# scitix/arks

Hardware: AMD Instinct MI355X
Metric: output_tok_s (higher is better)
Workload: dtype bf16; 1 GPU; model=qwen2.5-7b, global_batch=64, seq_len=1024, parallelism=dp1

## Files before the change

### arks_amd/ops/__init__.py

```python

from __future__ import annotations

import os
from typing import Callable, NamedTuple

import torch

from . import ref

_C = None
_C_ERR: str | None = None


def _load_extension():
    global _C, _C_ERR
    if _C is not None or _C_ERR is not None:
        return _C
    try:
        from . import _load

        _C = _load.C
    except Exception as e:
        _C_ERR = f"{type(e).__name__}: {e}"
    return _C
# ... 237 lines not shown
    return nparts


def attention_decode_paged(
    q, k_cache, v_cache, block_tables, seq_lens, scale: float,
    num_partitions: int | None = None, part_out=None, window: int = 0,
):
    if q.is_cuda:
        out = torch.empty(
            (q.shape[0], q.shape[1], q.shape[2]), dtype=q.dtype, device=q.device
        )
        num_kv_heads = k_cache.shape[1]
        if num_partitions is None:
            num_partitions = decode_num_partitions(
                q.shape[0], num_kv_heads, block_tables.shape[1]
            )
        if num_partitions > 1 and part_out is None:
            gq = q.shape[1] // num_kv_heads
            part_out = torch.empty(
                q.shape[0] * num_kv_heads * num_partitions * gq * (q.shape[2] + 2),
                dtype=torch.float32, device=q.device,
            )
        elif part_out is None:
            part_out = q.new_empty(0, dtype=torch.float32)
        _native().attention_decode_paged(
            out, q, k_cache, v_cache, block_tables, seq_lens, scale,
            part_out, num_partitions, window,
        )
        return out
    return ref.attention_decode_paged(
        q, k_cache, v_cache, block_tables, seq_lens, scale, window
    )


_EXTEND_WS: dict = {}


def _extend_ws(need: int, device):
    key = (device.index,)
    ws = _EXTEND_WS.get(key)
    if ws is None or ws.numel() < need:
        ws = torch.empty(need, dtype=torch.float32, device=device)
        _EXTEND_WS[key] = ws
    return ws


_SKINNY_WS: dict = {}
_SKINNY_WS_GEN: dict = {}


class SplitKPending:

    __slots__ = ("ws", "nsplits", "mrows", "shape", "bias", "_key", "_gen")

    def __init__(self, ws, nsplits, mrows, M, N, bias, key):
        self.ws = ws
        self.nsplits = nsplits
        self.mrows = mrows
        self.shape = (M, N)
        self.bias = bias
        self._key = key
        self._gen = _SKINNY_WS_GEN[key]

    def check_live(self) -> None:
        if _SKINNY_WS_GEN.get(self._key) != self._gen:
            raise RuntimeError(
                "stale split-K handle: another skinny GEMM has overwritten "
                "the shared workspace since this result was produced"
            )

    def materialize(self) -> torch.Tensor:
        self.check_live()
        out = torch.empty(self.shape, dtype=torch.bfloat16,
                          device=self.ws.device)
        _native().skinny_combine(out, self.ws, self.bias, self.nsplits,
                                 self.mrows)
        return out


def skinny_gemm(x, weight, bias=None, defer: bool = False):
    M, K = x.shape
    N = weight.shape[0]
    config, nsplits, k_per_split, mrows = _skinny_plan(M, N, K)
    part = (_skinny_ws(nsplits, N, mrows, x.device) if nsplits > 1
            else x.new_empty(0, dtype=torch.float32))
    if defer and nsplits > 1:
        _native().skinny_gemm_partials(part, x, weight, k_per_split, nsplits,
                                       config)
        return SplitKPending(part, nsplits, mrows, M, N, bias,
                             (x.device.index,))
    out = torch.empty((M, N), dtype=x.dtype, device=x.device)
    _native().skinny_gemm(out, part, x, weight, bias, k_per_split, nsplits,
                          config)
    return out


def _skinny_plan(M: int, N: int, K: int):
    ntiles = N // 64
    if K > N and ntiles < 128 and M > 48:
        config, mt = _SKINNY_TALLK_CONFIG, 4
        nsplits = min(-(-448 // ntiles), -(-K // 256))
    else:
        config, mt = 0, min(-(-M // 16), 4)
        nsplits = 1 if ntiles >= 384 else min(-(-512 // ntiles), -(-K // 256))
    k_per_split = -(-(-(-K // nsplits)) // 32) * 32
    nsplits = -(-K // k_per_split)
    return config, nsplits, k_per_split, 16 * mt


def _skinny_ws(nsplits: int, N: int, mrows: int, device):
    key = (device.index,)
    need = nsplits * N * mrows
    ws = _SKINNY_WS.get(key)
    if ws is None or ws.numel() < need:
        ws = torch.empty(need, dtype=torch.float32, device=device)
        _SKINNY_WS[key] = ws
    _SKINNY_WS_GEN[key] = _SKINNY_WS_GEN.get(key, 0) + 1
    return ws


_USE_SKINNY = os.environ.get("ARKS_SKINNY_GEMM", "1") == "1"
_SPLITK_FUSE = os.environ.get("ARKS_SPLITK_FUSE", "1") == "1"
_SKINNY_MAX_ELEMS = 34_000_000
_SKINNY_TALLK_MAX_ELEMS = 80_000_000
_TALLK_V = os.environ.get("ARKS_SKINNY_TALLK_V", "7").strip()
if _TALLK_V not in ("7", "8"):
    raise ValueError(
        f"ARKS_SKINNY_TALLK_V={_TALLK_V!r}: accepted values are 7 (tall-K "
        "kernel) and 8 (tall-K kernel with non-temporal W loads)"
    )
_SKINNY_TALLK_CONFIG = {"7": 1, "8": 2}[_TALLK_V]


def linear_bf16(x, weight, bias=None, defer: bool = False):
    if (
        _USE_SKINNY
        and x.is_cuda
        and x.dim() == 2
        and 1 <= x.shape[0] <= 64
        and x.dtype == torch.bfloat16
        and weight.shape[0] % 64 == 0
        and weight.shape[1] % 32 == 0
        and (weight.numel() <= _SKINNY_MAX_ELEMS
             or (weight.shape[1] > weight.shape[0]
                 and x.shape[0] > 48
                 and weight.numel() <= _SKINNY_TALLK_MAX_ELEMS))
        and weight.is_contiguous()
        and native_available()
    ):
        return skinny_gemm(x, weight, bias, defer=defer and _SPLITK_FUSE)
    import torch.nn.functional as F

    return F.linear(x, weight, bias)


W4_SKINNY_MAX_M = W8_SKINNY_MAX_M = _WQ_SKINNY_MAX_M = 64
W4_SLAB_MAX_M = 128
W8_SLAB_MAX_M = 128
_DEQUANT_WS: dict = {}


def reserve_dequant_workspace(numel: int, device) -> None:
    device = torch.device(device)
    if device.type != "cuda":
        return
    key = (device.index if device.index is not None
           else torch.cuda.current_device(),)
    ws = _DEQUANT_WS.get(key)
    if ws is None or ws.numel() < numel:
        _DEQUANT_WS[key] = torch.empty(numel, dtype=torch.bfloat16,
                                       device=device)


class _WqFormat(NamedTuple):
    name: str
    shape: Callable
    ref_linear: Callable
    ref_dequant: Callable
    slab_max_m: int


_W4 = _WqFormat(
    "w4", lambda w: (w[0].shape[0], w[0].shape[1] * 8), ref.w4_linear,
    lambda w: ref.w4_dequant(*ref.w4_unpack(w)), W4_SLAB_MAX_M)
_W8 = _WqFormat(
    "w8", lambda w: tuple(w[0].shape),
    lambda x, w, bias: ref.w8_linear(x, *w, bias),
    lambda w: ref.w8_dequant(*w), W8_SLAB_MAX_M)


# ... 388 lines not shown
```

### arks_amd/ops/csrc/bindings.cpp

```cpp
#include <torch/extension.h>

#include <c10/hip/HIPStream.h>
#include <hip/hip_runtime.h>

#include <cstring>
#include <string>
#include <vector>

namespace py = pybind11;

extern "C" {
void arks_rmsnorm(void* out, const void* input, const void* weight, float eps,
                  int rows, int hidden, hipStream_t stream);
void arks_fused_add_rmsnorm(void* out, const void* input, void* residual,
                            const void* weight, float eps, int rows, int hidden,
                            hipStream_t stream);
void arks_silu_mul(void* out, const void* gate_up, int64_t rows, int d,
                   hipStream_t stream);
int arks_pool_max_hidden();
void arks_pool_embed(void* out, void* carry, void* part, const void* x,
                     const void* residual, const void* weight,
                     const void* segs, const void* slabs, int nsegs,
                     int nslabs, float eps, int hidden, int dims,
                     int normalize, hipStream_t stream);
void arks_rope_inplace(const void* positions, void* q, void* k,
                       const void* cos_sin, int num_tokens, int head_dim,
                       int num_q_heads, int num_kv_heads, int64_t q_stride,
                       int64_t k_stride, hipStream_t stream);
void arks_reshape_and_cache(const void* k, const void* v, void* k_cache,
                            void* v_cache, const void* slot_mapping,
                            int num_tokens, int num_kv_heads, int head_dim,
                            int block_size, int64_t kv_stride, int kv_fp8,
                            hipStream_t stream);
void arks_rope_and_cache(const void* positions, void* q, void* k,
                         const void* v, void* k_cache, void* v_cache,
                         const void* slot_mapping, const void* cos_sin,
                         int num_tokens, int head_dim, int num_q_heads,
                         int num_kv_heads, int block_size, int64_t q_stride,
                         int64_t k_stride, int kv_fp8, hipStream_t stream);
void arks_attn_decode_paged(void* out, void* part_out, const void* q,
                            const void* k_cache, const void* v_cache,
                            const void* block_tables, const void* seq_lens,
                            float scale, int num_seqs, int num_q_heads,
                            int num_kv_heads, int head_dim, int max_blocks,
                            int nparts, int64_t q_stride, int kv_fp8,
                            int window, hipStream_t stream);
void arks_attn_prefill_varlen(void* out, const void* q, const void* k,
                              const void* v, const void* cu_seqlens,
                              const void* tile_info, int ntiles, float scale,
                              int num_q_heads, int num_kv_heads, int head_dim,
                              int64_t q_stride, int64_t kv_stride, int window,
                              hipStream_t stream);
void arks_attn_extend_paged(void* out, const void* q, const void* k_cache,
                            const void* v_cache, const void* block_tables,
                            const void* kv_lens, const void* cu_seqlens_q,
                            const void* tile_info, int ntiles, float scale,
                            int num_q_heads, int num_kv_heads, int head_dim,
                            int max_blocks, int64_t q_stride, int kv_fp8,
                            int window, hipStream_t stream);
void arks_attn_extend_paged2(void* out, const void* q, const void* k_cache,
                             const void* v_cache, const void* block_tables,
                             const void* kv_lens, const void* cu_seqlens_q,
                             const void* tile_info, void* part_ws, int ntiles,
                             float scale, int num_q_heads, int num_kv_heads,
                             int head_dim, int max_blocks, int64_t q_stride,
                             int window, hipStream_t stream);
void arks_attn_extend2_combine(void* out, const void* part_ws,
                               const void* combine_table,
                               const void* cu_seqlens_q, int n_split,
                               float scale, int num_q_heads, int head_dim,
                               hipStream_t stream);
void arks_quant_fp8_rows(void* out, void* inv_scale, const void* x, int rows,
                         int cols, hipStream_t stream);
void arks_rmsnorm_fp8(void* out, void* inv_scale, const void* input,
                      void* residual, const void* weight, float eps, int rows,
                      int hidden, int fused_add, hipStream_t stream);
void arks_silu_mul_fp8(void* out, void* inv_scale, const void* gate_up,
                       int rows, int d, hipStream_t stream);
void arks_skinny_gemm(void* part, void* out, const void* a, const void* w,
                      const void* bias, int m_rows, int n_total, int k_total,
                      int k_per_split, int nsplits, int64_t a_stride,
                      int config, bool combine, hipStream_t stream);
int arks_skinny_slab_rows(int m_rows, int config);
void arks_skinny_combine(void* out, const void* part, const void* bias,
                         int m_rows, int n_total, int nsplits, int mrows_pad,
                         hipStream_t stream);
void arks_splitk_add_rmsnorm(void* out, const void* part, const void* bias,
                             void* residual, const void* weight, float eps,
                             int rows, int hidden, int nsplits, int mrows_pad,
                             hipStream_t stream);
void arks_splitk_rope_and_cache(const void* positions, const void* part,
                                const void* bias, void* q_out, void* k_cache,
                                void* v_cache, const void* slot_mapping,
                                const void* cos_sin, int num_tokens,
                                int head_dim, int num_q_heads,
                                int num_kv_heads, int block_size, int nsplits,
                                int mrows_pad, int kv_fp8, hipStream_t stream);
void arks_greedy_sample(void* out, const void* logits, int rows, int vocab,
                        hipStream_t stream);
void arks_gumbel_sample(void* out, const void* logits, const void* temperatures,
                        const void* uniform, int rows, int vocab,
                        hipStream_t stream);
void arks_greedy_sample_masked(void* out, const void* logits,
                               const void* masks, const void* mask_row,
                               int rows, int vocab, int slots,
                               hipStream_t stream);
void arks_gumbel_sample_masked(void* out, const void* logits,
                               const void* temperatures, const void* uniform,
                               const void* masks, const void* mask_row,
                               int rows, int vocab, int slots,
                               hipStream_t stream);
void arks_apply_token_bitmask(void* logits, int is_fp32, const void* masks,
                              const void* mask_row, int rows, int vocab,
                              int slots, hipStream_t stream);
void arks_ar_seq_inc(void* seq, hipStream_t stream);
void arks_one_shot_allreduce(void* out, const void* src, void* mail_ptrs[8],
                             void* flag_ptrs[8], void* seq, int rank,
                             int world, int64_t n, hipStream_t stream);
void arks_moe_topk(void* weights, void* ids, const void* logits, int T,
                   int E, int k, int renorm, hipStream_t stream);
void arks_moe_mix(void* out, const void* y, const void* weights,
                  const void* ids, int T, int H, int k, int expert_base,
                  int n_local, hipStream_t stream);
void arks_moe_mix_rows(void* out, const void* y, const void* weights,
                       const void* rows, int T, int H, int k,
                       hipStream_t stream);
void arks_lora_shrink(void* h, const void* x, const void* a, const void* tiles,
                      int ntiles, int T, int K, int SR, int max_loras,
                      hipStream_t stream);
void arks_lora_expand(void* y, const void* h, const void* b, const void* tiles,
                      int ntiles, int T, int N, int R, int S, int off1,
                      int off2, int max_loras, hipStream_t stream);
void arks_w4_skinny_gemm(void* part, void* out, const void* a, const void* qw,
                         const void* scales, const void* zeros,
                         const void* bias, int m_rows, int n_total,
                         int k_total, int k_per_split, int nsplits,
                         int64_t a_stride, int nw, bool combine,
                         hipStream_t stream);
int arks_wq_slab_rows(int m_rows);
void arks_w4_dequant(void* out, const void* qw, const void* scales,
                     const void* zeros, int n_total, int k_total,
                     hipStream_t stream);
void arks_w4_moe_gemm(void* out, const void* a, const void* qw,
                      const void* scales, const void* zeros,
                      const void* counts, const void* pairs, int n_experts,
                      int t_cols, int n_pairs, int src_div, int slabs,
                      int n_total, int k_total, int nw, hipStream_t stream);
void arks_w8_skinny_gemm(void* part, void* out, const void* a, const void* w8,
                         const void* scales, const void* bias, int m_rows,
                         int n_total, int k_total, int k_per_split,
                         int nsplits, int64_t a_stride, int nw, bool combine,
                         hipStream_t stream);
void arks_w8_dequant(void* out, const void* w8, const void* scales,
                     int n_total, int k_total, hipStream_t stream);
void arks_moe_route(void* counts, void* pairs, const void* ids, int n_pairs,
                    int T, int expert_base, int n_local, hipStream_t stream);
void arks_mfma_probe(void* d, const void* a, const void* b, hipStream_t stream);
void arks_mfma_probe32(void* d, const void* a, const void* b, hipStream_t stream);
void arks_tr16_probe(void* out, int stride_bytes, hipStream_t stream);
}

namespace {

hipStream_t current_stream() {
  return c10::hip::getCurrentHIPStream().stream();
}
// ... 214 lines not shown
                             torch::Tensor cu_seqlens_q,
                             torch::Tensor tile_info, torch::Tensor part_ws,
                             double scale, int64_t window) {
  check_bf16_contig(out, "out");
  check_bf16_rowstrided(q, "q");
  check_bf16_contig(k_cache, "k_cache");
  check_bf16_contig(v_cache, "v_cache");
  TORCH_CHECK(block_tables.scalar_type() == torch::kInt32);
  TORCH_CHECK(kv_lens.scalar_type() == torch::kInt32);
  TORCH_CHECK(cu_seqlens_q.scalar_type() == torch::kInt32);
  TORCH_CHECK(tile_info.scalar_type() == torch::kInt32);
  TORCH_CHECK(tile_info.dim() == 2 && tile_info.size(1) == 4,
              "tile_info rows are (seq, q0, part, nparts)");
  const int num_q_heads = q.size(1);
  const int head_dim = q.size(2);
  const int num_kv_heads = k_cache.size(1);
  TORCH_CHECK(k_cache.size(2) == 16, "KV block size must be 16");
  TORCH_CHECK(head_dim == 64 || head_dim == 128, "head_dim must be 64 or 128");
  const int ntiles = tile_info.size(0);
  const int max_blocks = block_tables.size(1);
  void* ws = nullptr;
  if (part_ws.numel() > 0) {
    TORCH_CHECK(part_ws.scalar_type() == torch::kFloat32);
    ws = part_ws.data_ptr();
  }
  arks_attn_extend_paged2(out.data_ptr(), q.data_ptr(), k_cache.data_ptr(),
                          v_cache.data_ptr(), block_tables.data_ptr(),
                          kv_lens.data_ptr(), cu_seqlens_q.data_ptr(),
                          tile_info.data_ptr(), ws, ntiles, (float)scale,
                          num_q_heads, num_kv_heads, head_dim, max_blocks,
                          q.stride(0), (int)window, current_stream());
}

void attention_extend2_combine(torch::Tensor out, torch::Tensor part_ws,
                               torch::Tensor combine_table,
                               torch::Tensor cu_seqlens_q, double scale) {
  check_bf16_rowstrided(out, "out");
  TORCH_CHECK(part_ws.scalar_type() == torch::kFloat32);
  TORCH_CHECK(combine_table.scalar_type() == torch::kInt32 &&
              combine_table.dim() == 2 && combine_table.size(1) == 4);
  const int num_q_heads = out.size(1);
  const int head_dim = out.size(2);
  arks_attn_extend2_combine(out.data_ptr(), part_ws.data_ptr(),
                            combine_table.data_ptr(), cu_seqlens_q.data_ptr(),
                            combine_table.size(0), (float)scale, num_q_heads,
                            head_dim, current_stream());
}

const void* check_skinny_args(const torch::Tensor& out,
                              const torch::Tensor& part,
                              const torch::Tensor& a, const torch::Tensor& w,
                              const c10::optional<torch::Tensor>& bias,
                              int64_t k, int64_t nsplits, int64_t mrows,
                              bool partials_only, const char* what) {
  check_bf16_rowstrided(a, "a");
  check_bf16_contig(w, "w");
  const int64_t m = a.size(0), n = w.size(0);
  TORCH_CHECK(m >= 1 && m <= 64, what, " needs 1 <= M <= 64");
  TORCH_CHECK(n % 64 == 0 && k % 32 == 0, "N%64==0 and K%32==0 required");
  if (partials_only) {
    TORCH_CHECK(nsplits > 1, what, ": partials-only needs nsplits > 1");
  } else {
    check_bf16_contig(out, "out");
    TORCH_CHECK(out.size(0) == m && out.size(1) == n);
  }
  const void* bias_ptr = nullptr;
  if (bias.has_value()) {
    check_bf16_contig(*bias, "bias");
    TORCH_CHECK(bias->numel() == n);
    bias_ptr = bias->data_ptr();
  }
  if (nsplits > 1) {
    TORCH_CHECK(part.is_cuda() && part.scalar_type() == torch::kFloat32 &&
                part.is_contiguous() &&
                part.numel() >= (int64_t)nsplits * n * mrows,
                what, " workspace too small");
  }
  return bias_ptr;
}

void skinny_gemm_impl(torch::Tensor out, torch::Tensor part, torch::Tensor a,
                      torch::Tensor w, c10::optional<torch::Tensor> bias,
                      int64_t k_per_split, int64_t nsplits, int64_t config,
                      bool combine) {
  const int m = a.size(0), k = a.size(1), n = w.size(0);
  TORCH_CHECK(w.size(1) == k);
  TORCH_CHECK(0 <= config && config <= 2, "config in 0..2");
  TORCH_CHECK(k_per_split >= 32 && k_per_split % 32 == 0 &&
              nsplits * k_per_split >= k, "splits must cover K");
  const int mrows = arks_skinny_slab_rows(m, (int)config);
  const void* bias_ptr = check_skinny_args(out, part, a, w, bias, k, nsplits,
                                           mrows, !combine, "skinny_gemm");
  arks_skinny_gemm(nsplits > 1 ? part.data_ptr() : nullptr,
                   combine ? out.data_ptr() : nullptr, a.data_ptr(),
                   w.data_ptr(), bias_ptr, m, n, k, (int)k_per_split,
                   (int)nsplits, a.stride(0), (int)config, combine,
                   current_stream());
}

void skinny_gemm(torch::Tensor out, torch::Tensor part, torch::Tensor a,
                 torch::Tensor w, c10::optional<torch::Tensor> bias,
                 int64_t k_per_split, int64_t nsplits, int64_t config) {
  skinny_gemm_impl(out, part, a, w, bias, k_per_split, nsplits, config, true);
}

void skinny_gemm_partials(torch::Tensor part, torch::Tensor a, torch::Tensor w,
                          int64_t k_per_split, int64_t nsplits,
                          int64_t config) {
  skinny_gemm_impl(torch::Tensor(), part, a, w, c10::nullopt, k_per_split,
                   nsplits, config, false);
}

std::pair<int64_t, int64_t> check_w4_packed(const torch::Tensor& qw,
                                            const torch::Tensor& scales,
                                            const torch::Tensor& zeros) {
  TORCH_CHECK(qw.is_cuda() && qw.scalar_type() == torch::kInt32 &&
              qw.dim() == 2 && qw.is_contiguous(),
              "qweight must be contiguous int32 [N, K/8] on GPU");
  const int64_t n = qw.size(0), k = qw.size(1) * 8;
  TORCH_CHECK(k >= 128 && k % 128 == 0, "W4 needs K % 128 == 0, got K=", k);
  TORCH_CHECK(n % 64 == 0, "W4 needs N % 64 == 0, got N=", n);
  TORCH_CHECK(scales.is_cuda() && scales.scalar_type() == torch::kFloat16 &&
              scales.is_contiguous() && scales.dim() == 2 &&
              scales.size(0) == k / 128 && scales.size(1) == n,
              "scales must be contiguous f16 [K/128, N] on GPU");
  TORCH_CHECK(zeros.is_cuda() && zeros.scalar_type() == torch::kUInt8 &&
              zeros.is_contiguous() && zeros.dim() == 2 &&
              zeros.size(0) == k / 128 && zeros.size(1) == n,
              "zeros must be contiguous uint8 [K/128, N] on GPU");
  TORCH_CHECK(scales.device() == qw.device() && zeros.device() == qw.device());
  return {n, k};
}

struct WqSkinnyArgs {
  void* part;
  void* out;
  const void* bias;
};
WqSkinnyArgs check_wq_skinny(const torch::Tensor& out,
                             const torch::Tensor& part,
                             const torch::Tensor& a,
                             const c10::optional<torch::Tensor>& bias,
                             int64_t n, int64_t k, c10::Device dev,
                             int64_t k_per_split, int64_t nsplits, int64_t nw,
                             bool combine) {
  check_bf16_rowstrided(a, "a");
  TORCH_CHECK(a.dim() == 2 && a.size(1) == k, "a must be [M, K]");
  TORCH_CHECK(a.device() == dev);
  const int64_t m = a.size(0);
  TORCH_CHECK(m >= 1 && m <= 64, "wq_skinny_gemm needs 1 <= M <= 64");
  TORCH_CHECK(a.stride(0) % 8 == 0 &&
              reinterpret_cast<uintptr_t>(a.data_ptr()) % 16 == 0,
              "a rows must be 16-byte aligned");
  TORCH_CHECK((nw == 1 || nw == 2) && n % (64 * nw) == 0,
              "nw in {1, 2} with N % (64 * nw) == 0");
  TORCH_CHECK(nsplits >= 1 && k_per_split >= 128 && k_per_split % 128 == 0 &&
              nsplits * k_per_split >= k && (nsplits - 1) * k_per_split < k,
              "splits of a multiple of 128 must cover K exactly");
  WqSkinnyArgs r{nullptr, nullptr, nullptr};
  if (combine) {
    check_bf16_contig(out, "out");
    TORCH_CHECK(out.dim() == 2 && out.size(0) == m && out.size(1) == n);
    r.out = out.data_ptr();
    if (bias.has_value()) {
      check_bf16_contig(*bias, "bias");
      TORCH_CHECK(bias->numel() == n);
      r.bias = bias->data_ptr();
    }
  } else {
    TORCH_CHECK(nsplits > 1, "partials-only needs nsplits > 1");
  }
  if (nsplits > 1) {
    TORCH_CHECK(part.is_cuda() && part.scalar_type() == torch::kFloat32 &&
                part.is_contiguous() &&
                part.numel() >= nsplits * n * arks_wq_slab_rows((int)m) &&
                reinterpret_cast<uintptr_t>(part.data_ptr()) % 16 == 0,
                "wq_skinny_gemm workspace too small");
    r.part = part.data_ptr();
  }
  return r;
}

void w4_skinny_gemm_impl(torch::Tensor out, torch::Tensor part,
                         torch::Tensor a, torch::Tensor qw,
                         torch::Tensor scales, torch::Tensor zeros,
                         c10::optional<torch::Tensor> bias,
                         int64_t k_per_split, int64_t nsplits, int64_t nw,
                         bool combine) {
  const auto [n, k] = check_w4_packed(qw, scales, zeros);
  const auto p = check_wq_skinny(out, part, a, bias, n, k, qw.device(),
                                 k_per_split, nsplits, nw, combine);
  arks_w4_skinny_gemm(p.part, p.out, a.data_ptr(), qw.data_ptr(),
                      scales.data_ptr(), zeros.data_ptr(), p.bias,
// ... 560 lines not shown
                   (int)tiles.size(0), (int)T, (int)N, (int)R, (int)S,
                   S > 1 ? (int)slice_offsets[1] : (int)N,
                   S > 2 ? (int)slice_offsets[2] : (int)N, (int)b.size(0),
                   current_stream());
}

void pool_embed(torch::Tensor out, torch::Tensor carry, torch::Tensor part,
                torch::Tensor x, torch::Tensor residual, torch::Tensor weight,
                torch::Tensor segs, torch::Tensor slabs, double eps,
                int64_t dims, bool normalize) {
  check_bf16_contig(x, "x");
  check_bf16_contig(residual, "residual");
  check_bf16_contig(weight, "weight");
  TORCH_CHECK(x.dim() == 2 && x.sizes() == residual.sizes(),
              "x and residual are [T, H]");
  const int64_t H = x.size(1);
  TORCH_CHECK(H % 8 == 0, "pool_embed requires H % 8 == 0, got ", H);
  TORCH_CHECK(H <= arks_pool_max_hidden(), "pool_embed supports H <= ",
              arks_pool_max_hidden(), ", got ", H);
  TORCH_CHECK(weight.numel() == H, "weight must be [H]");
  TORCH_CHECK(dims >= 1 && dims <= H, "dims must be in [1, ", H, "], got ",
              dims);
  auto i32 = [](const torch::Tensor& t, int64_t cols, const char* name) {
    TORCH_CHECK(t.is_cuda() && t.scalar_type() == torch::kInt32 &&
                    t.is_contiguous() && t.dim() == 2 && t.size(1) == cols,
                name, " must be a contiguous int32 [n, ", cols, "] GPU tensor");
  };
  i32(segs, 8, "segs");
  i32(slabs, 4, "slabs");
  auto f32 = [](const torch::Tensor& t, const char* name) {
    TORCH_CHECK(t.is_cuda() && t.scalar_type() == torch::kFloat32 &&
                    t.is_contiguous(),
                name, " must be a contiguous f32 GPU tensor");
  };
  f32(out, "out");
  f32(carry, "carry");
  f32(part, "part");
  const int64_t S = segs.size(0), NS = slabs.size(0);
  TORCH_CHECK(S >= 1, "empty segment table");
  TORCH_CHECK(out.dim() == 2 && out.size(0) == S && out.size(1) == dims,
              "out must be [num_segments, dims]");
  TORCH_CHECK(carry.dim() == 2 && carry.size(1) == H, "carry must be [slots, H]");
  TORCH_CHECK(part.numel() >= NS * H, "partial workspace too small");
  check_align16(x, "x");
  check_align16(residual, "residual");
  check_align16(weight, "weight");
  if (NS > 0) check_align16(part, "part");
  if (carry.numel() > 0) check_align16(carry, "carry");
  arks_pool_embed(out.data_ptr(), carry.data_ptr(), part.data_ptr(),
                  x.data_ptr(), residual.data_ptr(), weight.data_ptr(),
                  segs.data_ptr(), slabs.data_ptr(), (int)S, (int)NS,
                  (float)eps, (int)H, (int)dims, normalize ? 1 : 0,
                  current_stream());
}

void mfma_probe(torch::Tensor d, torch::Tensor a, torch::Tensor b) {
  check_bf16_contig(a, "a");
  check_bf16_contig(b, "b");
  TORCH_CHECK(d.scalar_type() == torch::kFloat32 && d.is_contiguous());
  TORCH_CHECK(a.size(0) == 16 && a.size(1) == 32);
  TORCH_CHECK(b.size(0) == 32 && b.size(1) == 16);
  arks_mfma_probe(d.data_ptr(), a.data_ptr(), b.data_ptr(), current_stream());
}

}

PYBIND11_MODULE(TORCH_EXTENSION_NAME, m) {
  m.def("rmsnorm", &rmsnorm);
  m.def("fused_add_rmsnorm", &fused_add_rmsnorm);
  m.def("silu_mul", &silu_mul);
  m.def("rope_inplace", &rope_inplace);
  m.def("reshape_and_cache", &reshape_and_cache);
  m.def("rope_and_cache", &rope_and_cache);
  m.def("attention_decode_paged", &attention_decode_paged);
  m.def("attention_prefill_varlen", &attention_prefill_varlen);
  m.def("attention_extend_paged", &attention_extend_paged);
  m.def("attention_extend_paged2", &attention_extend_paged2);
  m.def("attention_extend2_combine", &attention_extend2_combine);
  m.def("quant_fp8_rows", &quant_fp8_rows);
  m.def("rmsnorm_fp8", &rmsnorm_fp8);
  m.def("silu_mul_fp8", &silu_mul_fp8);
  m.def("skinny_gemm", &skinny_gemm, py::arg("out"), py::arg("part"),
        py::arg("a"), py::arg("w"), py::arg("bias"), py::arg("k_per_split"),
        py::arg("nsplits"), py::arg("config") = 0);
  m.def("skinny_gemm_partials", &skinny_gemm_partials, py::arg("part"),
        py::arg("a"), py::arg("w"), py::arg("k_per_split"),
        py::arg("nsplits"), py::arg("config") = 0);
  m.def("skinny_combine", &skinny_combine);
  m.def("w4_skinny_gemm", &w4_skinny_gemm);
  m.def("w4_skinny_gemm_partials", &w4_skinny_gemm_partials);
  m.def("w4_dequant", &w4_dequant);
  m.def("w4_moe_gemm", &w4_moe_gemm);
  m.def("w8_skinny_gemm", &w8_skinny_gemm);
  m.def("w8_skinny_gemm_partials", &w8_skinny_gemm_partials);
  m.def("w8_dequant", &w8_dequant);
  m.def("splitk_add_rmsnorm", &splitk_add_rmsnorm);
  m.def("splitk_rope_and_cache", &splitk_rope_and_cache);
  m.def("greedy_sample", &greedy_sample);
  m.def("gumbel_sample", &gumbel_sample);
  m.def("greedy_sample_masked", &greedy_sample_masked);
  m.def("gumbel_sample_masked", &gumbel_sample_masked);
  m.def("apply_token_bitmask", &apply_token_bitmask);
  m.def("ipc_alloc", &ipc_alloc);
  m.def("arm_flags", &arm_flags);
  m.def("ipc_alloc_free", &ipc_alloc_free);
  m.def("ipc_handle", &ipc_handle);
  m.def("ipc_open", &ipc_open);
  m.def("ipc_close", &ipc_close);
  m.def("one_shot_allreduce", &one_shot_allreduce);
  m.def("moe_topk", &moe_topk);
  m.def("moe_route", &moe_route);
  m.def("moe_mix", &moe_mix);
  m.def("moe_mix_rows", &moe_mix_rows);
  m.def("lora_shrink", &lora_shrink);
  m.def("lora_expand", &lora_expand);
  m.def("pool_embed", &pool_embed);
  m.def("mfma_probe", &mfma_probe);
  m.def("mfma_probe32", &mfma_probe32);
  m.def("tr16_probe", &tr16_probe);
}
```

### arks_amd/ops/csrc/elementwise.hip

```cpp
#include "common.h"

namespace arks {

__device__ __forceinline__ float add_square(const float ss, const float v) {
#pragma clang fp contract(off)
  return ss + v * v;
}

constexpr int NORM_BLOCK = 256;

__device__ __forceinline__ float add_residual8(const ushort8 x,
                                               bf16* __restrict__ res,
                                               float ss) {
  ushort8 r = *reinterpret_cast<const ushort8*>(res);
  ushort8 s;
#pragma unroll
  for (int j = 0; j < 8; ++j) {
    float v = bf16_bits_to_float(x[j]) + bf16_bits_to_float(r[j]);
    s[j] = float_to_bf16_bits(v);
    ss = add_square(ss, bf16_bits_to_float(s[j]));
  }
  *reinterpret_cast<ushort8*>(res) = s;
  return ss;
}

__device__ __forceinline__ void rmsnorm_finish(bf16* __restrict__ out_row,
                                               const bf16* __restrict__ src_row,
                                               const bf16* __restrict__ weight,
                                               const float ss, const float eps,
                                               const int hidden) {
  __shared__ float red[NORM_BLOCK / WAVE_SIZE];
  float total = block_reduce_sum<NORM_BLOCK>(ss, red);
  const float rrms = rsqrtf(total / (float)hidden + eps);
  for (int i = threadIdx.x; i < hidden / 8; i += NORM_BLOCK) {
    ushort8 x = *reinterpret_cast<const ushort8*>(src_row + i * 8);
    ushort8 w = *reinterpret_cast<const ushort8*>(weight + i * 8);
    ushort8 o;
#pragma unroll
    for (int j = 0; j < 8; ++j) {
      float v = bf16_bits_to_float(x[j]) * rrms * bf16_bits_to_float(w[j]);
      o[j] = float_to_bf16_bits(v);
    }
    *reinterpret_cast<ushort8*>(out_row + i * 8) = o;
  }
}

template <bool FUSED_ADD>
__global__ void rmsnorm_kernel(bf16* __restrict__ out,
                               const bf16* __restrict__ input,
                               bf16* __restrict__ residual,
                               const bf16* __restrict__ weight,
                               const float eps, const int hidden) {
  const int row = blockIdx.x;
  const bf16* in_row = input + (int64_t)row * hidden;
  bf16* res_row = FUSED_ADD ? residual + (int64_t)row * hidden : nullptr;

  const int nvec = hidden / 8;
  float ss = 0.f;
  for (int i = threadIdx.x; i < nvec; i += NORM_BLOCK) {
    ushort8 x = *reinterpret_cast<const ushort8*>(in_row + i * 8);
    if constexpr (FUSED_ADD) {
      ss = add_residual8(x, res_row + i * 8, ss);
    } else {
#pragma unroll
      for (int j = 0; j < 8; ++j) {
        float v = bf16_bits_to_float(x[j]);
        ss += v * v;
      }
    }
  }
  rmsnorm_finish(out + (int64_t)row * hidden, FUSED_ADD ? res_row : in_row,
                 weight, ss, eps, hidden);
}

__global__ __launch_bounds__(256) void splitk_add_rmsnorm_kernel(
    bf16* __restrict__ out, const float* __restrict__ part,
    const bf16* __restrict__ bias,
    bf16* __restrict__ residual, const bf16* __restrict__ weight,
    const float eps, const int hidden, const int nsplits,
    const int64_t split_stride) {
  const int row = blockIdx.x;
  const float* part_row = part + (int64_t)row * hidden;
  bf16* res_row = residual + (int64_t)row * hidden;

  const int nvec = hidden / 8;
  float ss = 0.f;
  for (int i = threadIdx.x; i < nvec; i += NORM_BLOCK) {
    const float* const p[2] = {part_row + i * 8, part_row + i * 8 + 4};
    float4v acc[2];
    splitk_reduce<2, 2>(p, split_stride, nsplits, acc);
    ushort8 x;
#pragma unroll
    for (int j = 0; j < 8; ++j) {
      float xf = acc[j / 4][j % 4];
      if (bias != nullptr) xf += bf16_bits_to_float(bias[i * 8 + j]);
      x[j] = float_to_bf16_bits(xf);
    }
    ss = add_residual8(x, res_row + i * 8, ss);
  }
  rmsnorm_finish(out + (int64_t)row * hidden, res_row, weight, ss, eps,
                 hidden);
}

__global__ void silu_mul_kernel(bf16* __restrict__ out,
                                const bf16* __restrict__ gate_up,
                                const int d, const int64_t total_vec) {
  for (int64_t idx = (int64_t)blockIdx.x * blockDim.x + threadIdx.x;
       idx < total_vec; idx += (int64_t)gridDim.x * blockDim.x) {
    const int64_t row = idx / (d / 8);
    const int col8 = (int)(idx % (d / 8)) * 8;
    const bf16* g = gate_up + row * (2 * (int64_t)d) + col8;
    const bf16* u = g + d;
    ushort8 gv = *reinterpret_cast<const ushort8*>(g);
    ushort8 uv = *reinterpret_cast<const ushort8*>(u);
    ushort8 o;
#pragma unroll
    for (int j = 0; j < 8; ++j) {
      float x = bf16_bits_to_float(gv[j]);
      float silu = x / (1.f + __expf(-x));
      o[j] = float_to_bf16_bits(silu * bf16_bits_to_float(uv[j]));
    }
    *reinterpret_cast<ushort8*>(out + row * d + col8) = o;
  }
}

__global__ void rope_kernel(const int64_t* __restrict__ positions,
                            bf16* __restrict__ q, bf16* __restrict__ k,
                            const float* __restrict__ cos_sin,
                            const int head_dim, const int num_q_heads,
                            const int num_kv_heads, const int64_t q_stride,
                            const int64_t k_stride) {
  const int token = blockIdx.x;
  const int half = head_dim / 2;
  const int64_t pos = positions[token];
  const float* cs = cos_sin + pos * head_dim;
  const int total_heads = num_q_heads + num_kv_heads;
  const int pairs2 = half / 2;
  for (int idx = threadIdx.x; idx < total_heads * pairs2; idx += blockDim.x) {
    const int h = idx / pairs2;
    const int p2 = (idx % pairs2) * 2;
    bf16* base = (h < num_q_heads)
                     ? q + (int64_t)token * q_stride + (int64_t)h * head_dim
                     : k + (int64_t)token * k_stride +
                           (int64_t)(h - num_q_heads) * head_dim;
    ushort2v x1 = *reinterpret_cast<const ushort2v*>(base + p2);
    ushort2v x2 = *reinterpret_cast<const ushort2v*>(base + half + p2);
    ushort2v o1, o2;
#pragma unroll
    for (int j = 0; j < 2; ++j) {
      uint16_t r1, r2;
      rope_rotate(bf16_bits_to_float(x1[j]), bf16_bits_to_float(x2[j]),
                  cs[p2 + j], cs[half + p2 + j], r1, r2);
      o1[j] = r1;
      o2[j] = r2;
    }
    *reinterpret_cast<ushort2v*>(base + p2) = o1;
    *reinterpret_cast<ushort2v*>(base + half + p2) = o2;
  }
}

}

using namespace arks;

extern "C" {

void arks_rmsnorm(void* out, const void* input, const void* weight, float eps,
                  int rows, int hidden, hipStream_t stream) {
  dim3 grid(rows), block(256);
  hipLaunchKernelGGL((rmsnorm_kernel<false>), grid, block, 0, stream,
                     (bf16*)out, (const bf16*)input, nullptr,
                     (const bf16*)weight, eps, hidden);
}

void arks_fused_add_rmsnorm(void* out, const void* input, void* residual,
                            const void* weight, float eps, int rows, int hidden,
                            hipStream_t stream) {
  dim3 grid(rows), block(256);
  hipLaunchKernelGGL((rmsnorm_kernel<true>), grid, block, 0, stream, (bf16*)out,
                     (const bf16*)input, (bf16*)residual, (const bf16*)weight,
                     eps, hidden);
}

void arks_splitk_add_rmsnorm(void* out, const void* part, const void* bias,
                             void* residual, const void* weight, float eps,
                             int rows, int hidden, int nsplits, int mrows_pad,
                             hipStream_t stream) {
  dim3 grid(rows), block(256);
  hipLaunchKernelGGL(splitk_add_rmsnorm_kernel, grid, block, 0, stream,
                     (bf16*)out, (const float*)part, (const bf16*)bias,
                     (bf16*)residual, (const bf16*)weight, eps, hidden,
                     nsplits, (int64_t)mrows_pad * hidden);
}

void arks_silu_mul(void* out, const void* gate_up, int64_t rows, int d,
                   hipStream_t stream) {
  int64_t total_vec = rows * (d / 8);
  int blocks = (int)std::min<int64_t>((total_vec + 255) / 256, 2048);
  if (blocks == 0) blocks = 1;
  hipLaunchKernelGGL(silu_mul_kernel, dim3(blocks), dim3(256), 0, stream,
                     (bf16*)out, (const bf16*)gate_up, d, total_vec);
}

void arks_rope_inplace(const void* positions, void* q, void* k,
                       const void* cos_sin, int num_tokens, int head_dim,
                       int num_q_heads, int num_kv_heads, int64_t q_stride,
                       int64_t k_stride, hipStream_t stream) {
  dim3 grid(num_tokens), block(256);
  hipLaunchKernelGGL(rope_kernel, grid, block, 0, stream,
                     (const int64_t*)positions, (bf16*)q, (bf16*)k,
                     (const float*)cos_sin, head_dim, num_q_heads,
                     num_kv_heads, q_stride, k_stride);
}

}
```

### arks_amd/ops/csrc/skinny_gemm.hip

```cpp
#include "common.h"

#include <algorithm>
#include <cfloat>
#include <type_traits>

namespace arks {

typedef __attribute__((ext_vector_type(8))) __bf16 bf16x8;
typedef __attribute__((ext_vector_type(4))) float f32x4;

__device__ __forceinline__ f32x4 sk_mfma(bf16x8 a, bf16x8 b, f32x4 c) {
  return __builtin_amdgcn_mfma_f32_16x16x32_bf16(a, b, c, 0, 0, 0);
}

constexpr int SK_AP = 8;

template <int MT>
__device__ __forceinline__ void store_partials(float* __restrict__ part,
                                               const f32x4 (&acc)[MT],
                                               const int n_total,
                                               const int n, const int lq) {
  float* p = part + (int64_t)blockIdx.y * (16 * MT) * n_total + n;
#pragma unroll
  for (int t = 0; t < MT; ++t)
    *reinterpret_cast<f32x4*>(p + (int64_t)(t * 16 + lq) * n_total) = acc[t];
}

constexpr int SK_KC = 128;
constexpr int SK_D = 4;

template <int MT, bool NT = false, int WAVES = 4>
__global__ __launch_bounds__(64 * WAVES, 2) void skinny_gemm_kernel(
    float* __restrict__ part,
    bf16* __restrict__ out,
    const bf16* __restrict__ a,
    const bf16* __restrict__ w,
    const bf16* __restrict__ bias,
    const int m_rows, const int n_total, const int k_total,
    const int k_per_split, const int nsplits, const int64_t a_stride) {
  constexpr int KC = SK_KC;
  constexpr int D = SK_D;
  constexpr int KSTEPS = KC / 32;
  constexpr int CPT = KC / 8;
  constexpr int THREADS = 64 * WAVES;
  constexpr int NTW = 16 * WAVES;
  constexpr int RPP = THREADS / CPT;
  constexpr int NIT = 16 * MT / RPP;
  static_assert(D % 2 == 0, "LDS slot parity follows the ring slot");
  static_assert(NIT * RPP == 16 * MT, "A chunk must divide over the threads");
  const int n0 = blockIdx.x * NTW;
  const int kb = blockIdx.y * k_per_split;
  const int ke = min(k_total, kb + k_per_split);
  const int klen = max(ke - kb, 0);
  const int nch = (klen + KC - 1) / KC;

  const int tid = threadIdx.x;
  const int wave = tid / WAVE_SIZE;
  const int lane = tid % WAVE_SIZE;
  const int lq = lane % 16;
  const int la = lane / 16;

  __shared__ __attribute__((aligned(16))) union {
    bf16 a_buf[2][64][KC + SK_AP];
    float c_buf[NTW][64 + 1];
  } lds;

  f32x4 acc[MT];
#pragma unroll
  for (int t = 0; t < MT; ++t) acc[t] = {0.f, 0.f, 0.f, 0.f};

  const bool wave_live = n0 + wave * 16 < n_total;
  const bf16* wrow =
      w + (int64_t)min(n0 + wave * 16 + lq, n_total - 1) * k_total + 8 * la;

  const int acol = (tid % CPT) * 8;
  const bf16* arow[NIT];
#pragma unroll
  for (int it = 0; it < NIT; ++it)
    arow[it] = a + (int64_t)min(tid / CPT + it * RPP, m_rows - 1) * a_stride;

  ushort8 wreg[D][KSTEPS];
  ushort8 areg[D][NIT];

  auto issue = [&](int ch, ushort8 (&wd)[KSTEPS], ushort8 (&ad)[NIT],
                   bool live) {
// ... 33 lines not shown
        acc[t] = sk_mfma(wfrag, *reinterpret_cast<bf16x8*>(&af), acc[t]);
      }
    }
  };

#pragma unroll
  for (int p = 0; p < D; ++p) {
    issue(p, wreg[p], areg[p], p < nch);
    __builtin_amdgcn_sched_barrier(0);
  }
  write_a(areg[0], 0);
  __syncthreads();

  int c = 0;
  auto ring_turn = [&](auto nrefill) {
    constexpr int R = decltype(nrefill)::value;
#pragma unroll
    for (int s = 0; s < D; ++s) {
      mfma_chunk(wreg[s], s & 1, KC);
      __builtin_amdgcn_sched_barrier(0);
      if (s < R) issue(c + D + s, wreg[s], areg[s], true);
      __builtin_amdgcn_sched_barrier(0);
      if (s + 1 < D || R > 0) {
        write_a(areg[(s + 1) % D], (s + 1) & 1);
        __syncthreads();
      }
    }
    c += D;
  };
  auto drain = [&](auto nleft) {
    constexpr int R = decltype(nleft)::value;
#pragma unroll
    for (int s = 0; s < R; ++s) {
      mfma_chunk(wreg[s], s & 1, s + 1 < R ? KC : klen - (c + s) * KC);
      if (s + 1 < R) {
        write_a(areg[s + 1], (s + 1) & 1);
        __syncthreads();
      }
    }
  };
  using std::integral_constant;
  while (c + 2 * D <= nch) ring_turn(integral_constant<int, D>{});
  switch (nch - c) {
    case 7: ring_turn(integral_constant<int, 3>{});
            drain(integral_constant<int, 3>{}); break;
    case 6: ring_turn(integral_constant<int, 2>{});
            drain(integral_constant<int, 2>{}); break;
    case 5: ring_turn(integral_constant<int, 1>{});
            drain(integral_constant<int, 1>{}); break;
    case 4: drain(integral_constant<int, 4>{}); break;
    case 3: drain(integral_constant<int, 3>{}); break;
    case 2: drain(integral_constant<int, 2>{}); break;
    case 1: drain(integral_constant<int, 1>{}); break;
    default: break;
  }
  static_assert(D == 4, "the tail switch is written out for D = 4");

  if (nsplits > 1) {
    if (wave_live)
      store_partials<MT>(part, acc, n_total, n0 + wave * 16 + 4 * la, lq);
    return;
  }

  __syncthreads();
#pragma unroll
  for (int t = 0; t < MT; ++t) {
#pragma unroll
    for (int r = 0; r < 4; ++r) {
      lds.c_buf[wave * 16 + 4 * la + r][t * 16 + lq] = acc[t][r];
    }
  }
  __syncthreads();
  const int nvalid = min(NTW, n_total - n0);
  for (int i = tid; i < m_rows * NTW; i += THREADS) {
    const int m = i / NTW;
    const int n = i % NTW;
    if (n >= nvalid) continue;
    float v = lds.c_buf[n][m];
    if (bias != nullptr) v += bf16_bits_to_float(bias[n0 + n]);
    out[(int64_t)m * n_total + n0 + n] = float_to_bf16_bits(v);
  }
}

__global__ __launch_bounds__(256) void skinny_combine_kernel(
    bf16* __restrict__ out, const float* __restrict__ part,
    const bf16* __restrict__ bias, const int m_rows, const int n_total,
    const int nsplits, const int64_t split_stride) {
  const int nq = n_total / 4;
  const int i = blockIdx.x * 256 + threadIdx.x;
  if (i >= m_rows * nq) return;
  const int m = i / nq;
  const int n = (i % nq) * 4;
  const float* const p[1] = {part + (int64_t)m * n_total + n};
  float4v s[1];
  splitk_reduce<1, 2>(p, split_stride, nsplits, s);
  ushort4v o;
#pragma unroll
  for (int e = 0; e < 4; ++e) {
    float v = s[0][e];
    if (bias != nullptr) v += bf16_bits_to_float(bias[n + e]);
    o[e] = float_to_bf16_bits(v);
  }
  *reinterpret_cast<ushort4v*>(out + (int64_t)m * n_total + n) = o;
}

}

using namespace arks;

extern "C" void arks_skinny_combine(void* out, const void* part,
                                    const void* bias, int m_rows, int n_total,
                                    int nsplits, int mrows_pad,
                                    hipStream_t stream) {
  dim3 cgrid((m_rows * (n_total / 4) + 255) / 256), cblock(256);
  hipLaunchKernelGGL(skinny_combine_kernel, cgrid, cblock, 0, stream,
                     (bf16*)out, (const float*)part, (const bf16*)bias, m_rows,
                     n_total, nsplits, (int64_t)mrows_pad * n_total);
}

static int skinny_mt(int m_rows, int config) {
  return config == 0 ? std::min((m_rows + 15) / 16, 4) : 4;
}

extern "C" int arks_skinny_slab_rows(int m_rows, int config) {
  return 16 * skinny_mt(m_rows, config);
}

extern "C" void arks_skinny_gemm(void* part, void* out, const void* a,
                                 const void* w, const void* bias, int m_rows,
                                 int n_total, int k_total, int k_per_split,
                                 int nsplits, int64_t a_stride, int config,
                                 bool combine, hipStream_t stream) {
  const int waves = config == 0 ? 4 : 8;
  dim3 grid((n_total + 16 * waves - 1) / (16 * waves), nsplits);
  dim3 block(64 * waves);
  auto launch = [&](auto kernel) {
    hipLaunchKernelGGL(kernel, grid, block, 0, stream, (float*)part,
                       (bf16*)out, (const bf16*)a, (const bf16*)w,
                       (const bf16*)bias, m_rows, n_total, k_total,
                       k_per_split, nsplits, a_stride);
  };
  if (config == 2) {
    launch(skinny_gemm_kernel<4, true, 8>);
  } else if (config == 1) {
    launch(skinny_gemm_kernel<4, false, 8>);
  } else {
    switch (skinny_mt(m_rows, config)) {
      case 1: launch(skinny_gemm_kernel<1>); break;
      case 2: launch(skinny_gemm_kernel<2>); break;
      case 3: launch(skinny_gemm_kernel<3>); break;
      default: launch(skinny_gemm_kernel<4>); break;
    }
  }
  if (nsplits > 1 && combine)
    arks_skinny_combine(out, part, bias, m_rows, n_total, nsplits,
                        arks_skinny_slab_rows(m_rows, config), stream);
}
```

Before: 11630 tok/s.

## Add persistent A-resident split-K skinny GEMM and wide split-K add-rmsnorm kernel

Adds a new skinny GEMM path (config 3) in which each workgroup stages its K-slice of the activation into LDS once. It then streams many 16-column weight slabs through a register ring buffer, with the grid sized to the CU count divided by the number of splits. This is meant to cut repeated activation loads and launch/tile overhead for split-K decode GEMMs with short per-split K. It also adds a 512-thread variant of the split-K add+rmsnorm that covers the whole hidden row with one vector per thread. The trade-offs are reduced parallelism per launch and LDS pressure.

```diff
diff --git a/arks_amd/ops/__init__.py b/arks_amd/ops/__init__.py
--- a/arks_amd/ops/__init__.py
+++ b/arks_amd/ops/__init__.py
@@ -343,6 +343,7 @@
     M, K = x.shape
     N = weight.shape[0]
     config, nsplits, k_per_split, mrows = _skinny_plan(M, N, K)
+    config = _skinny_resident_config(config, M, nsplits, k_per_split)
     part = (_skinny_ws(nsplits, N, mrows, x.device) if nsplits > 1
             else x.new_empty(0, dtype=torch.float32))
     if defer and nsplits > 1:
@@ -367,6 +368,20 @@
     k_per_split = -(-(-(-K // nsplits)) // 32) * 32
     nsplits = -(-K // k_per_split)
     return config, nsplits, k_per_split, 16 * mt
+
+
+_SKINNY_RESIDENT_KMAX = 512
+_SKINNY_RESIDENT = os.environ.get("ARKS_SKINNY_RESIDENT", "1") == "1"
+_SKINNY_RESIDENT_MIN_M = 1
+
+
+def _skinny_resident_config(config: int, M: int, nsplits: int,
+                            k_per_split: int) -> int:
+    if (_SKINNY_RESIDENT and config == 0 and nsplits > 1
+            and k_per_split <= _SKINNY_RESIDENT_KMAX
+            and M >= _SKINNY_RESIDENT_MIN_M):
+        return 3
+    return config
 
 
 def _skinny_ws(nsplits: int, N: int, mrows: int, device):
diff --git a/arks_amd/ops/csrc/bindings.cpp b/arks_amd/ops/csrc/bindings.cpp
--- a/arks_amd/ops/csrc/bindings.cpp
+++ b/arks_amd/ops/csrc/bindings.cpp
@@ -80,8 +80,10 @@
 void arks_skinny_gemm(void* part, void* out, const void* a, const void* w,
                       const void* bias, int m_rows, int n_total, int k_total,
                       int k_per_split, int nsplits, int64_t a_stride,
-                      int config, bool combine, hipStream_t stream);
+                      int config, bool combine, hipStream_t stream,
+                      int groups);
 int arks_skinny_slab_rows(int m_rows, int config);
+int arks_skinny_resident_kmax();
 void arks_skinny_combine(void* out, const void* part, const void* bias,
                          int m_rows, int n_total, int nsplits, int mrows_pad,
                          hipStream_t stream);
@@ -462,12 +464,18 @@
 void skinny_gemm_impl(torch::Tensor out, torch::Tensor part, torch::Tensor a,
                       torch::Tensor w, c10::optional<torch::Tensor> bias,
                       int64_t k_per_split, int64_t nsplits, int64_t config,
-                      bool combine) {
+                      int64_t groups, bool combine) {
   const int m = a.size(0), k = a.size(1), n = w.size(0);
   TORCH_CHECK(w.size(1) == k);
-  TORCH_CHECK(0 <= config && config <= 2, "config in 0..2");
+  TORCH_CHECK(0 <= config && config <= 3, "config in 0..3");
   TORCH_CHECK(k_per_split >= 32 && k_per_split % 32 == 0 &&
               nsplits * k_per_split >= k, "splits must cover K");
+  TORCH_CHECK(config != 3 ||
+                  (nsplits > 1 && k_per_split <= arks_skinny_resident_kmax()),
+              "config 3 needs nsplits > 1 and k_per_split <= ",
+              arks_skinny_resident_kmax());
+  TORCH_CHECK(0 <= groups && groups <= 65535, "groups in 0..65535");
+  TORCH_CHECK(nsplits <= 65535, "too many splits");
   const int mrows = arks_skinny_slab_rows(m, (int)config);
   const void* bias_ptr = check_skinny_args(out, part, a, w, bias, k, nsplits,
                                            mrows, !combine, "skinny_gemm");
@@ -475,20 +483,22 @@
                    combine ? out.data_ptr() : nullptr, a.data_ptr(),
                    w.data_ptr(), bias_ptr, m, n, k, (int)k_per_split,
                    (int)nsplits, a.stride(0), (int)config, combine,
-                   current_stream());
+                   current_stream(), (int)groups);
 }
 
 void skinny_gemm(torch::Tensor out, torch::Tensor part, torch::Tensor a,
                  torch::Tensor w, c10::optional<torch::Tensor> bias,
-                 int64_t k_per_split, int64_t nsplits, int64_t config) {
-  skinny_gemm_impl(out, part, a, w, bias, k_per_split, nsplits, config, true);
+                 int64_t k_per_split, int64_t nsplits, int64_t config,
+                 int64_t groups) {
+  skinny_gemm_impl(out, part, a, w, bias, k_per_split, nsplits, config, groups,
+                   true);
 }
 
 void skinny_gemm_partials(torch::Tensor part, torch::Tensor a, torch::Tensor w,
                           int64_t k_per_split, int64_t nsplits,
-                          int64_t config) {
+                          int64_t config, int64_t groups) {
   skinny_gemm_impl(torch::Tensor(), part, a, w, c10::nullopt, k_per_split,
-                   nsplits, config, false);
+                   nsplits, config, groups, false);
 }
 
 std::pair<int64_t, int64_t> check_w4_packed(const torch::Tensor& qw,
@@ -1215,10 +1225,10 @@
   m.def("silu_mul_fp8", &silu_mul_fp8);
   m.def("skinny_gemm", &skinny_gemm, py::arg("out"), py::arg("part"),
         py::arg("a"), py::arg("w"), py::arg("bias"), py::arg("k_per_split"),
-        py::arg("nsplits"), py::arg("config") = 0);
+        py::arg("nsplits"), py::arg("config") = 0, py::arg("groups") = 0);
   m.def("skinny_gemm_partials", &skinny_gemm_partials, py::arg("part"),
         py::arg("a"), py::arg("w"), py::arg("k_per_split"),
-        py::arg("nsplits"), py::arg("config") = 0);
+        py::arg("nsplits"), py::arg("config") = 0, py::arg("groups") = 0);
   m.def("skinny_combine", &skinny_combine);
   m.def("w4_skinny_gemm", &w4_skinny_gemm);
   m.def("w4_skinny_gemm_partials", &w4_skinny_gemm_partials);
diff --git a/arks_amd/ops/csrc/elementwise.hip b/arks_amd/ops/csrc/elementwise.hip
--- a/arks_amd/ops/csrc/elementwise.hip
+++ b/arks_amd/ops/csrc/elementwise.hip
@@ -100,6 +100,76 @@
   }
   rmsnorm_finish(out + (int64_t)row * hidden, res_row, weight, ss, eps,
                  hidden);
+}
+
+constexpr int NORM_WIDE_BLOCK = 512;
+
+__global__ __launch_bounds__(NORM_WIDE_BLOCK) void splitk_add_rmsnorm_wide_kernel(
+    bf16* __restrict__ out, const float* __restrict__ part,
+    const bf16* __restrict__ bias,
+    bf16* __restrict__ residual, const bf16* __restrict__ weight,
+    const float eps, const int hidden, const int nsplits,
+    const int64_t split_stride) {
+  __shared__ struct {
+    ushort8 hi[NORM_WIDE_BLOCK - NORM_BLOCK];
+    float red[NORM_BLOCK / WAVE_SIZE];
+  } lds;
+  const int row = blockIdx.x;
+  const int tid = threadIdx.x;
+  const int nvec = hidden / 8;
+  const bool live = tid < nvec;
+  const int col = live ? tid * 8 : 0;
+  const float* part_row = part + (int64_t)row * hidden;
+  bf16* res = residual + (int64_t)row * hidden + col;
+
+  const ushort8 r = *reinterpret_cast<const ushort8*>(res);
+  const ushort8 w = *reinterpret_cast<const ushort8*>(weight + col);
+  ushort8 b = {0, 0, 0, 0, 0, 0, 0, 0};
+  if (bias != nullptr) b = *reinterpret_cast<const ushort8*>(bias + col);
+  const float* const p[2] = {part_row + col, part_row + col + 4};
+  float4v acc[2];
+  splitk_reduce<2, 2>(p, split_stride, nsplits, acc);
+
+  ushort8 s;
+#pragma unroll
+  for (int j = 0; j < 8; ++j) {
+    float xf = acc[j / 4][j % 4];
+    if (bias != nullptr) xf += bf16_bits_to_float(b[j]);
+    const uint16_t x = float_to_bf16_bits(xf);
+    s[j] = float_to_bf16_bits(bf16_bits_to_float(x) +
+                              bf16_bits_to_float(r[j]));
+  }
+  if (live) *reinterpret_cast<ushort8*>(res) = s;
+  if (tid >= NORM_BLOCK) lds.hi[tid - NORM_BLOCK] = s;
+  __syncthreads();
+
+  if (tid < NORM_BLOCK) {
+    float ss = 0.f;
+    if (live) {
+#pragma unroll
+      for (int j = 0; j < 8; ++j) ss = add_square(ss, bf16_bits_to_float(s[j]));
+    }
+    if (tid + NORM_BLOCK < nvec) {
+      const ushort8 h = lds.hi[tid];
+#pragma unroll
+      for (int j = 0; j < 8; ++j) ss = add_square(ss, bf16_bits_to_float(h[j]));
+    }
+    ss = wave_reduce_sum(ss);
+    if (tid % WAVE_SIZE == 0) lds.red[tid / WAVE_SIZE] = ss;
+  }
+  __syncthreads();
+  float total = 0.f;
+#pragma unroll
+  for (int wv = 0; wv < NORM_BLOCK / WAVE_SIZE; ++wv) total += lds.red[wv];
+  const float rrms = rsqrtf(total / (float)hidden + eps);
+  if (!live) return;
+  ushort8 o;
+#pragma unroll
+  for (int j = 0; j < 8; ++j) {
+    float v = bf16_bits_to_float(s[j]) * rrms * bf16_bits_to_float(w[j]);
+    o[j] = float_to_bf16_bits(v);
+  }
+  *reinterpret_cast<ushort8*>(out + (int64_t)row * hidden + col) = o;
 }
 
 __global__ void silu_mul_kernel(bf16* __restrict__ out,
@@ -186,11 +256,13 @@
                              void* residual, const void* weight, float eps,
                              int rows, int hidden, int nsplits, int mrows_pad,
                              hipStream_t stream) {
-  dim3 grid(rows), block(256);
-  hipLaunchKernelGGL(splitk_add_rmsnorm_kernel, grid, block, 0, stream,
-                     (bf16*)out, (const float*)part, (const bf16*)bias,
-                     (bf16*)residual, (const bf16*)weight, eps, hidden,
-                     nsplits, (int64_t)mrows_pad * hidden);
+  const bool wide = hidden <= 8 * NORM_WIDE_BLOCK;
+  dim3 grid(rows), block(wide ? NORM_WIDE_BLOCK : NORM_BLOCK);
+  hipLaunchKernelGGL(
+      wide ? splitk_add_rmsnorm_wide_kernel : splitk_add_rmsnorm_kernel, grid,
+      block, 0, stream, (bf16*)out, (const float*)part, (const bf16*)bias,
+      (bf16*)residual, (const bf16*)weight, eps, hidden, nsplits,
+      (int64_t)mrows_pad * hidden);
 }
 
 void arks_silu_mul(void* out, const void* gate_up, int64_t rows, int d,
diff --git a/arks_amd/ops/csrc/skinny_gemm.hip b/arks_amd/ops/csrc/skinny_gemm.hip
--- a/arks_amd/ops/csrc/skinny_gemm.hip
+++ b/arks_amd/ops/csrc/skinny_gemm.hip
@@ -1,6 +1,7 @@
 #include "common.h"
 
 #include <algorithm>
+#include <atomic>
 #include <cfloat>
 #include <type_traits>
 
@@ -200,6 +201,153 @@
   }
 }
 
+constexpr int SKR_WAVES = 4;
+constexpr int SKR_KMAX = 512;
+
+template <int MT>
+__global__ __launch_bounds__(64 * SKR_WAVES, 2) void skinny_resident_kernel(
+    float* __restrict__ part,
+    const bf16* __restrict__ a,
+    const bf16* __restrict__ w,
+    const int m_rows, const int n_total, const int k_total,
+    const int k_per_split, const int64_t a_stride, const int slabs_per_group) {
+  constexpr int KC = SK_KC;
+  constexpr int WAVES = SKR_WAVES;
+  constexpr int NA = 16 * MT / WAVES;
+  static_assert(NA * WAVES == 16 * MT, "A rows must divide over the waves");
+  extern __shared__ __attribute__((aligned(16))) bf16 a_lds[];
+  const int lstride = k_per_split + SK_AP;
+
+  const int kb = blockIdx.y * k_per_split;
+  const int ke = min(k_total, kb + k_per_split);
+  const int klen = max(ke - kb, 0);
+  const int nch = (klen + KC - 1) / KC;
+
+  const int tid = threadIdx.x;
+  const int wave = tid / WAVE_SIZE;
+  const int lane = tid % WAVE_SIZE;
+  const int lq = lane % 16;
+  const int la = lane / 16;
+
+  const int slab0 = blockIdx.x * slabs_per_group;
+  const int nwg = max(min(slabs_per_group, n_total / 16 - slab0), 0);
+  const int nsl = (nwg - wave + WAVES - 1) / WAVES;
+
+  ushort8 areg[NA];
+  const int lcol = max(min(8 * lane, klen - 8), 0);
+  const int acol = min(kb + lcol, k_total - 8);
+  auto load_a = [&]() {
+#pragma unroll
+    for (int it = 0; it < NA; ++it)
+      areg[it] = *reinterpret_cast<const ushort8*>(
+          a + (int64_t)min(it * WAVES + wave, m_rows - 1) * a_stride + acol);
+    __builtin_amdgcn_sched_barrier(0);
+  };
+  auto stage_a = [&]() {
+#pragma unroll
+    for (int it = 0; it < NA; ++it)
+      *reinterpret_cast<ushort8*>(
+          &a_lds[(it * WAVES + wave) * lstride + lcol]) = areg[it];
+    __syncthreads();
+  };
+
+  const bf16* wlane = w + 8 * la;
+  const bf16* afrag = a_lds + lq * lstride + 8 * la;
+  using std::integral_constant;
+
+  auto stream = [&](auto nch_c) {
+    constexpr int NCH = decltype(nch_c)::value;
+    constexpr int KS = NCH * (KC / 32);
+    constexpr int R = NCH >= 3 ? 2 : 3;
+    ushort8 wreg[R][KS];
+
+    auto issue = [&](int i, ushort8 (&wd)[KS], bool live) {
+      const bf16* wrow =
+          wlane +
+          (int64_t)((slab0 + wave + i * WAVES) * 16 + lq) * k_total;
+#pragma unroll
+      for (int s = 0; s < KS; ++s) {
+        const bf16* src = wrow + min(kb + s * 32, k_total - 32);
+        wd[s] = *reinterpret_cast<const ushort8*>(live ? src : w);
+      }
+    };
+    auto consume = [&](int i, const ushort8 (&wd)[KS]) {
+      f32x4 acc[MT];
+#pragma unroll
+      for (int t = 0; t < MT; ++t) acc[t] = {0.f, 0.f, 0.f, 0.f};
+#pragma unroll
+      for (int s = 0; s < KS; ++s) {
+        if (s >= KS - KC / 32 && s * 32 >= klen) break;
+        ushort8 wv = wd[s];
+        bf16x8 wfrag = *reinterpret_cast<bf16x8*>(&wv);
+#pragma unroll
+        for (int t = 0; t < MT; ++t) {
+          ushort8 af = *reinterpret_cast<const ushort8*>(
+              afrag + t * 16 * lstride + s * 32);
+          acc[t] = sk_mfma(wfrag, *reinterpret_cast<bf16x8*>(&af), acc[t]);
+        }
+      }
+      store_partials<MT>(part, acc, n_total,
+                         (slab0 + wave + i * WAVES) * 16 + 4 * la, lq);
+    };
+
+    asm volatile("; resident path, %0 chunks" ::"n"(NCH));
+    load_a();
+#pragma unroll
+    for (int p = 0; p < R; ++p) {
+      issue(p, wreg[p], p < nsl);
+      __builtin_amdgcn_sched_barrier(0);
+    }
+    stage_a();
+    __builtin_amdgcn_sched_barrier(0);
+
+    int c = 0;
+    auto ring_turn = [&](auto nrefill) {
+      constexpr int NR = decltype(nrefill)::value;
+#pragma unroll
+      for (int s = 0; s < R; ++s) {
+        consume(c + s, wreg[s]);
+        __builtin_amdgcn_sched_barrier(0);
+        if (s < NR) issue(c + R + s, wreg[s], true);
+        __builtin_amdgcn_sched_barrier(0);
+      }
+      c += R;
+    };
+    auto drain = [&](auto nleft) {
+      constexpr int NL = decltype(nleft)::value;
+#pragma unroll
+      for (int s = 0; s < NL; ++s) consume(c + s, wreg[s]);
+    };
+    auto tail = [&](auto rem) {
+      constexpr int REM = decltype(rem)::value;
+      if constexpr (REM >= 2 * R) {
+      } else if constexpr (REM >= R) {
+        ring_turn(integral_constant<int, REM - R>{});
+        drain(integral_constant<int, REM - R>{});
+      } else {
+        drain(integral_constant<int, REM>{});
+      }
+    };
+    while (c + 2 * R <= nsl) ring_turn(integral_constant<int, R>{});
+    switch (nsl - c) {
+      case 5: tail(integral_constant<int, 5>{}); break;
+      case 4: tail(integral_constant<int, 4>{}); break;
+      case 3: tail(integral_constant<int, 3>{}); break;
+      case 2: tail(integral_constant<int, 2>{}); break;
+      case 1: tail(integral_constant<int, 1>{}); break;
+      default: break;
+    }
+    static_assert(R <= 3, "the tail switch is written out for R <= 3");
+  };
+
+  switch (nch) {
+    case 4: stream(integral_constant<int, 4>{}); break;
+    case 3: stream(integral_constant<int, 3>{}); break;
+    case 2: stream(integral_constant<int, 2>{}); break;
+    default: stream(integral_constant<int, 1>{}); break;
+  }
+}
+
 __global__ __launch_bounds__(256) void skinny_combine_kernel(
     bf16* __restrict__ out, const float* __restrict__ part,
     const bf16* __restrict__ bias, const int m_rows, const int n_total,
@@ -237,18 +385,73 @@
 }
 
 static int skinny_mt(int m_rows, int config) {
-  return config == 0 ? std::min((m_rows + 15) / 16, 4) : 4;
+  return config == 0 || config == 3 ? std::min((m_rows + 15) / 16, 4) : 4;
 }
 
 extern "C" int arks_skinny_slab_rows(int m_rows, int config) {
   return 16 * skinny_mt(m_rows, config);
+}
+
+extern "C" int arks_skinny_resident_kmax() { return SKR_KMAX; }
+
+static int device_cu_count() {
+  constexpr int MAX_DEV = 64;
+  static std::atomic<int> cus[MAX_DEV];
+  int dev = 0;
+  if (hipGetDevice(&dev) != hipSuccess || dev < 0 || dev >= MAX_DEV) dev = 0;
+  int n = cus[dev].load(std::memory_order_relaxed);
+  if (n == 0) {
+    if (hipDeviceGetAttribute(&n, hipDeviceAttributeMultiprocessorCount,
+                              dev) != hipSuccess || n <= 0)
+      n = 1;
+    cus[dev].store(n, std::memory_order_relaxed);
+  }
+  return n;
+}
+
+template <int MT>
+static void launch_resident(float* part, const bf16* a, const bf16* w,
+                            int m_rows, int n_total, int k_total,
+                            int k_per_split, int nsplits, int64_t a_stride,
+                            int groups, hipStream_t stream) {
+  const int slabs = n_total / 16;
+  if (groups <= 0)
+    groups = std::min(std::max(device_cu_count() / nsplits, 1), slabs);
+  const int per_group = (slabs + groups - 1) / groups;
+  const size_t lds = (size_t)16 * MT * (k_per_split + SK_AP) * sizeof(bf16);
+  if (lds > 64 * 1024)
+    (void)hipFuncSetAttribute(
+        reinterpret_cast<const void*>(&skinny_resident_kernel<MT>),
+        hipFuncAttributeMaxDynamicSharedMemorySize,
+        16 * MT * (SKR_KMAX + SK_AP) * (int)sizeof(bf16));
+  hipLaunchKernelGGL(skinny_resident_kernel<MT>, dim3(groups, nsplits),
+                     dim3(64 * SKR_WAVES), lds, stream, part, a, w, m_rows,
+                     n_total, k_total, k_per_split, a_stride, per_group);
 }
 
 extern "C" void arks_skinny_gemm(void* part, void* out, const void* a,
                                  const void* w, const void* bias, int m_rows,
                                  int n_total, int k_total, int k_per_split,
                                  int nsplits, int64_t a_stride, int config,
-                                 bool combine, hipStream_t stream) {
+                                 bool combine, hipStream_t stream,
+                                 int groups = 0) {
+  if (config == 3) {
+    auto launch = [&](auto mt) {
+      launch_resident<decltype(mt)::value>(
+          (float*)part, (const bf16*)a, (const bf16*)w, m_rows, n_total,
+          k_total, k_per_split, nsplits, a_stride, groups, stream);
+    };
+    switch (skinny_mt(m_rows, config)) {
+      case 1: launch(std::integral_constant<int, 1>{}); break;
+      case 2: launch(std::integral_constant<int, 2>{}); break;
+      case 3: launch(std::integral_constant<int, 3>{}); break;
+      default: launch(std::integral_constant<int, 4>{}); break;
+    }
+    if (combine)
+      arks_skinny_combine(out, part, bias, m_rows, n_total, nsplits,
+                          arks_skinny_slab_rows(m_rows, config), stream);
+    return;
+  }
   const int waves = config == 0 ? 4 : 8;
   dim3 grid((n_total + 16 * waves - 1) / (16 * waves), nsplits);
   dim3 block(64 * waves);
```

After: 12060 tok/s (median of 6 runs). 1.04x the previous value.
